# PREDICT-EPFL/piqp

Hardware: AMD Instinct MI355X
Metric: KKT factor+solve/sec (per IPM iter) (higher is better)
Workload: dtype f64; 1 GPU; dense QP n=4096 p=0 m_ineq=4096 (BASELINE configs[1]), kkt_solver=dense_cholesky, 1 update_scalings_and_factor + 2 KKTSystem::solve per step, inputs resident in HBM; n=4096, p=0, m=4096, parallelism=independent QP replicas x1

## Files before the change

piqp_amd/csrc/dense_kernels.hip:

```cpp
#include "dense_kernels.hpp"

#include <algorithm>
#include <map>
#include <mutex>
#include <stdexcept>
#include <type_traits>
#include <utility>
#include <vector>
#include <cstdlib>
#include <cstdio>
#include <cstring>

namespace pq {
namespace dense {

typedef double d4 __attribute__((ext_vector_type(4)));
typedef double d2 __attribute__((ext_vector_type(2)));

__device__ __forceinline__ double readlane_d(double v, int srclane)
{
    long long bits = __double_as_longlong(v);
    int lo = (int)(bits & 0xffffffffll), hi = (int)(bits >> 32);
    lo = __builtin_amdgcn_readlane(lo, srclane);
    hi = __builtin_amdgcn_readlane(hi, srclane);
// ... 595 lines not shown
    if (!front_panel(j, panel, k, nb, rs) || rs <= 0) return;
    const int T = (rs + TS - 1) / TS;
    const int b = (int)blockIdx.x / SPLIT, h = (int)blockIdx.x % SPLIT;
    if (b >= T * (T + 1) / 2) return;
    int ti = (int)((sqrt(8.0 * (double)b + 1.0) - 1.0) * 0.5);
    while ((ti + 1) * (ti + 2) / 2 <= b) ++ti;
    while (ti * (ti + 1) / 2 > b) --ti;
    const int tj = b - ti * (ti + 1) / 2;
    if (ti * TS + (TS / SPLIT) * h >= rs) return;
    SyrkArgs a;
    a.n = rs; a.kdim = nb;
    a.A = j.F + (k + nb) + (size_t)k * j.f; a.lda = j.f; a.B = a.A; a.ldb = j.f; a.w = j.dvec + k;
    a.C = j.F + (k + nb) + (size_t)(k + nb) * j.f; a.ldc = j.f;
    a.unaligned = ((j.f & 1) || (reinterpret_cast<uintptr_t>(a.A) & 15)) ? 1 : 0;
    if (j.multi) {
        a.ncol = j.w - (k + nb);
        if (a.ncol <= 0 || tj * TS >= a.ncol) return;
    }
    extern __shared__ __attribute__((aligned(16))) double smem[];
    (void)fused_tile<512, false, true, true, SPLIT == 4>(a, ti, tj, smem, h);
}

template <int EPI>
__global__ __launch_bounds__(256) void k_syrk_tail_reduce(SyrkArgs a)
{
    const int b = a.tile_begin + (int)blockIdx.x;
    int ti, tj;
    if (a.tile_order) {
        const int pk = a.tile_order[b];
        ti = pk >> 16; tj = pk & 0xffff;
    } else {
        ti = (int)((sqrt(8.0 * (double)b + 1.0) - 1.0) * 0.5);
        while ((ti + 1) * (ti + 2) / 2 <= b) ++ti;
        while (ti * (ti + 1) / 2 > b) --ti;
        tj = b - ti * (ti + 1) / 2;
    }
    const int row0 = ti * TS, col0 = tj * TS;
    const double* P0 = a.part + (size_t)blockIdx.x * a.k_split * TS * TS;
    {
        const int idx = (int)blockIdx.y * 256 + (int)threadIdx.x;
        const int li = idx & (TS - 1), lj = idx >> 7;
        const int gi = row0 + li, gj = col0 + lj;
        if (gi >= a.n || gj >= a.n || gi < gj) return;
        double v = 0.0;
#pragma unroll 8
        for (int sl = 0; sl < a.k_split; ++sl) v += P0[(size_t)sl * TS * TS + idx];
        const size_t ci = (size_t)gi + (size_t)gj * a.ldc;
        if (EPI == EPI_ASSEMBLE) {
            double base = a.Pfull[(size_t)gi + (size_t)gj * a.ldp];
            if (gi == gj) base += a.x_reg[gi];
            if (a.ATA) base += a.dinv * a.ATA[(size_t)gi + (size_t)gj * a.ldata];
            a.C[ci] = base + v;
        } else if (EPI == EPI_SUBTRACT) {
            a.C[ci] -= v;
        } else {
            a.C[ci] = v;
        }
    }
}

static int g_slots = 0;
static int syrk_slots()
{
    if (g_slots == 0) {
        int dev = 0, cus = 256;
        if (hipGetDevice(&dev) == hipSuccess) (void)hipDeviceGetAttribute(&cus, hipDeviceAttributeMultiprocessorCount, dev);
        g_slots = 2 * (cus > 0 ? cus : 256);
    }
    return g_slots;
}
static void syrk_tail_plan(int n, int kdim, int& rem, int& ksplit)
{
    const int T = div_up(n, TS);
    const int ntiles = T * (T + 1) / 2;
    const int slots = syrk_slots();
    const int nkt = div_up(kdim, BK);
    rem = ntiles % slots;
    ksplit = 1;
    if (ntiles > slots && rem > 0 && rem * 10 < slots * 6) {
        int s = slots / rem;
        s = std::min(s, nkt / 4);
        if (s >= 2) ksplit = s;
// ... 12 lines not shown
    bool low_latency;
    bool tile_order;
    int rem, k_split;
};
static bool syrk_wants_tile_order(int T) { return T >= 16; }
static SyrkPlan syrk_plan(int n, int kdim, bool with_ws, size_t ws_doubles)
{
    SyrkPlan p;
    p.T = div_up(n, TS);
    p.ntiles = p.T * (p.T + 1) / 2;
    p.rem = 0; p.k_split = 1;
    if (with_ws) syrk_tail_plan(n, kdim, p.rem, p.k_split);
    if (p.rem > 0 && (size_t)p.rem * p.k_split * TS * TS > ws_doubles) { p.rem = 0; p.k_split = 1; }
    p.low_latency = kdim <= 256;
    p.tile_order = !p.low_latency && syrk_wants_tile_order(p.T);
    return p;
}
void syrk_debug_plan(int n, int kdim, bool with_workspace, int out[6])
{
    const SyrkPlan p = syrk_plan(n, kdim, with_workspace, ~(size_t)0);
    out[0] = p.T; out[1] = p.ntiles; out[2] = p.low_latency ? 1 : 0; out[3] = p.tile_order ? 1 : 0; out[4] = p.rem; out[5] = p.k_split;
}

static const int* syrk_tile_order(int T)
{
    static std::mutex mu;
    static std::map<std::pair<int, int>, int*> cache;
    if (!syrk_wants_tile_order(T)) return nullptr;
    int dev = 0;
    if (hipGetDevice(&dev) != hipSuccess) return nullptr;
    std::lock_guard<std::mutex> lk(mu);
    auto it = cache.find({dev, T});
    if (it != cache.end()) return it->second;
    constexpr int S = 8, NX = 8;
    std::vector<int> blocked;
    for (int SI = 0; SI * S < T; ++SI)
        for (int SJ = 0; SJ <= SI; ++SJ)
            for (int ti = SI * S; ti < std::min(T, SI * S + S); ++ti)
                for (int tj = SJ * S; tj < SJ * S + S && tj <= ti; ++tj) blocked.push_back(ti << 16 | tj);
    const int nt = (int)blocked.size();
    std::vector<int> start(NX + 1, 0);
    for (int x = 0; x < NX; ++x) start[x + 1] = start[x] + nt / NX + (x < nt % NX ? 1 : 0);
    std::vector<int> order(nt);
    for (int b = 0; b < nt; ++b) order[b] = blocked[start[b % NX] + b / NX];
    int* d = nullptr;
    if (hipMalloc(&d, sizeof(int) * nt) != hipSuccess) { (void)hipGetLastError(); cache[{dev, T}] = nullptr; return nullptr; }
    ++alloc_counter();
    if (hipMemcpy(d, order.data(), sizeof(int) * nt, hipMemcpyHostToDevice) != hipSuccess) { (void)hipGetLastError(); (void)hipFree(d); d = nullptr; }
    cache[{dev, T}] = d;
    return d;
}

void syrk_prepare(int n) { (void)syrk_tile_order(div_up(n, TS)); }

template <int EPI>
static void launch_syrk_t(SyrkArgs a, hipStream_t s, double* ws, size_t ws_doubles)
{
    const SyrkPlan pl = syrk_plan(a.n, a.kdim, ws != nullptr, ws_doubles);
    const int main_tiles = pl.ntiles - pl.rem;
    a.tile_begin = 0; a.k_split = 1; a.part = nullptr;
    a.tile_order = pl.tile_order ? syrk_tile_order(pl.T) : nullptr;
    if (pl.low_latency) hipLaunchKernelGGL((k_syrk_lower<EPI, 4, 4>), dim3(main_tiles), dim3(1024), SYRK_LDS_BYTES, s, a);
    else hipLaunchKernelGGL((k_syrk_lower<EPI, 2, 2>), dim3(main_tiles), dim3(256), SYRK_LDS_BYTES, s, a);
    if (pl.rem > 0) {
        a.tile_begin = main_tiles; a.k_split = pl.k_split; a.part = ws;
        hipLaunchKernelGGL((k_syrk_lower<EPI, 2, 2>), dim3(pl.rem * pl.k_split), dim3(256), SYRK_LDS_BYTES, s, a);
        hipLaunchKernelGGL(k_syrk_tail_reduce<EPI>, dim3(pl.rem, TS * TS / 256), dim3(256), 0, s, a);
    }
}

void launch_syrk(int epi, const SyrkArgs& args_in, hipStream_t s, double* split_ws, size_t split_ws_doubles)
{
    SyrkArgs a = args_in;
    if (a.n <= 0) return;
    a.unaligned = ((a.lda & 1) || (a.ldb & 1) || (reinterpret_cast<uintptr_t>(a.A) & 15) || (reinterpret_cast<uintptr_t>(a.B) & 15)) ? 1 : 0;
    static PerDeviceOnce attr_set;
    attr_set([&] {
        PQ_HIP(hipFuncSetAttribute(reinterpret_cast<const void*>(k_syrk_lower<EPI_ASSEMBLE, 2, 2>), hipFuncAttributeMaxDynamicSharedMemorySize, SYRK_LDS_BYTES));
        PQ_HIP(hipFuncSetAttribute(reinterpret_cast<const void*>(k_syrk_lower<EPI_SUBTRACT, 2, 2>), hipFuncAttributeMaxDynamicSharedMemorySize, SYRK_LDS_BYTES));
        PQ_HIP(hipFuncSetAttribute(reinterpret_cast<const void*>(k_syrk_lower<EPI_STORE, 2, 2>), hipFuncAttributeMaxDynamicSharedMemorySize, SYRK_LDS_BYTES));
        PQ_HIP(hipFuncSetAttribute(reinterpret_cast<const void*>(k_syrk_lower<EPI_ASSEMBLE, 4, 4>), hipFuncAttributeMaxDynamicSharedMemorySize, SYRK_LDS_BYTES));
        PQ_HIP(hipFuncSetAttribute(reinterpret_cast<const void*>(k_syrk_lower<EPI_SUBTRACT, 4, 4>), hipFuncAttributeMaxDynamicSharedMemorySize, SYRK_LDS_BYTES));
        PQ_HIP(hipFuncSetAttribute(reinterpret_cast<const void*>(k_syrk_lower<EPI_STORE, 4, 4>), hipFuncAttributeMaxDynamicSharedMemorySize, SYRK_LDS_BYTES));
    });
    if (epi == EPI_SUBTRACT_POTRF) {
        static PerDeviceOnce fused_attr;
        fused_attr([&] {
            PQ_HIP(hipFuncSetAttribute(reinterpret_cast<const void*>(k_syrk_lower<EPI_SUBTRACT_POTRF, 4, 2>), hipFuncAttributeMaxDynamicSharedMemorySize, FUSED_LDS_BYTES));
        });
        const int T = div_up(a.n, TS);
        a.tile_begin = 0; a.k_split = 1; a.part = nullptr;
        if (!a.fuse_scratch || !a.fuse_flags || a.fuse_nb <= 0 || a.kdim > TS) throw std::runtime_error("fused trailing update: scratch / flags / panel width");
        hipLaunchKernelGGL((k_syrk_lower<EPI_SUBTRACT_POTRF, 4, 2>), dim3(T * (T + 1) / 2 + FUSE_ROLES - 1), dim3(512), FUSED_LDS_BYTES, s, a);
        PQ_HIP(hipGetLastError());
        return;
    }
    switch (epi) {
    case EPI_ASSEMBLE: launch_syrk_t<EPI_ASSEMBLE>(a, s, split_ws, split_ws_doubles); break;
    case EPI_SUBTRACT: launch_syrk_t<EPI_SUBTRACT>(a, s, split_ws, split_ws_doubles); break;
    default: launch_syrk_t<EPI_STORE>(a, s, split_ws, split_ws_doubles); break;
    }
    PQ_HIP(hipGetLastError());
}

__global__ __launch_bounds__(256) void k_assemble_no_g(int n, const double* __restrict__ Pf, const double* __restrict__ x_reg, const double* __restrict__ ATA, double dinv, double* __restrict__ C)
{
    const int j = blockIdx.y;
    const int i = blockIdx.x * 256 + threadIdx.x;
    if (i < n && i >= j) {
        double v = Pf[i + (size_t)j * n];
        if (i == j) v += x_reg[i];
        if (ATA) v += dinv * ATA[i + (size_t)j * n];
        C[i + (size_t)j * n] = v;
    }
}
void launch_assemble_no_g(int n, const double* Pf, const double* x_reg, const double* ATA, double dinv, double* C, hipStream_t s)
{
    if (n <= 0) return;
    hipLaunchKernelGGL(k_assemble_no_g, dim3(div_up(n, 256), n), dim3(256), 0, s, n, Pf, x_reg, ATA, dinv, C);
    PQ_HIP(hipGetLastError());
}


// ... 357 lines not shown
    const int tid = threadIdx.x, lane = tid & 63, wave = tid >> 6;
    for (int b = wave; b < TB_BLOCKS; b += POTRF_THREADS / 64) {
        int bi = 0;
        while ((bi + 1) * (bi + 2) / 2 <= b) ++bi;
        const int bj = b - bi * (bi + 1) / 2;
        double v[4];
#pragma unroll
        for (int q = 0; q < 4; ++q) {
            const int e = lane + 64 * q, r = 16 * bi + (e & 15), c = 16 * bj + (e >> 4);
            const bool in = r < nb && c < nb;
            const bool ok = in && r >= c;
            const double* p = ok ? (A + r + (size_t)c * lda) : A;
            const double t = *p;
            v[q] = ok ? t : ((!in && r == c) ? 1.0 : 0.0);
        }
#pragma unroll
        for (int q = 0; q < 4; ++q) Tb[b * 256 + lane + 64 * q] = v[q];
    }
    __syncthreads();
    potrf_block<LDLT, POTRF_THREADS / 64>(Tb, Tb + TB_DOUBLES, nb, kglobal, info, rdiag, dvec, A, lda, pack, w16, ts, cnt, nactive, nullptr, nullptr, 0, nullptr, pack_lkk);
}
template <bool LDLT>
__global__ __launch_bounds__(POTRF_THREADS) void k_potrf_diag(double* __restrict__ A, int lda, int nb, int kglobal, int* __restrict__ info, double* __restrict__ rdiag,
                                                              double* __restrict__ dvec, double* __restrict__ pack, double* __restrict__ w16, long long* __restrict__ ts)
{
    potrf_diag_body<LDLT>(A, lda, nb, kglobal, info, rdiag, dvec, pack, w16, ts);
}
__global__ __launch_bounds__(POTRF_THREADS) void k_potrf_diag_fronts(const FrontJob* __restrict__ jobs, int panel, int* __restrict__ info, double* __restrict__ rdiag)
{
    const FrontJob j = jobs[blockIdx.x];
    int k, nb, rs;
    if (j.kind != 0 || !front_panel(j, panel, k, nb, rs)) return;
    potrf_diag_body<true>(j.F + k + (size_t)k * j.f, j.f, nb, j.first + k, info, rdiag, j.dvec + k, rs > 0 ? j.pack : nullptr, nullptr, nullptr, min(8, (nb + 15) >> 4));
}

void launch_potrf_diag(bool ldlt, double* A, int lda, int nb, int kglobal, int* info, double* rdiag, double* dvec, double* pack, double* w16, hipStream_t s, long long* ts)
{
    static PerDeviceOnce attr_set;
    attr_set([&] {
        PQ_HIP(hipFuncSetAttribute(reinterpret_cast<const void*>(k_potrf_diag<false>), hipFuncAttributeMaxDynamicSharedMemorySize, POTRF_LDS_BYTES));
        PQ_HIP(hipFuncSetAttribute(reinterpret_cast<const void*>(k_potrf_diag<true>), hipFuncAttributeMaxDynamicSharedMemorySize, POTRF_LDS_BYTES));
    });
    if (ldlt) hipLaunchKernelGGL(k_potrf_diag<true>, dim3(1), dim3(POTRF_THREADS), POTRF_LDS_BYTES, s, A, lda, nb, kglobal, info, rdiag, dvec, pack, w16, ts);
    else hipLaunchKernelGGL(k_potrf_diag<false>, dim3(1), dim3(POTRF_THREADS), POTRF_LDS_BYTES, s, A, lda, nb, kglobal, info, rdiag, dvec, pack, w16, ts);
    PQ_HIP(hipGetLastError());
}

template <int NT, bool PERSIST>
__device__ __forceinline__ bool fused_next_diag(const SyrkArgs& a, double* __restrict__ smem, int role)
{
    constexpr int NW = NT / 64;
    static_assert(FUSE_OWN * FUSE_ROLES >= TB_BLOCKS && FUSE_OWN <= NW, "every tile block needs a wave");
    double* As = smem;
    const int tid = threadIdx.x, lane = tid & 63, wave = tid >> 6;
    const int i = lane & 15, g = lane >> 4;
    const bool dbg_ts = FUSE_TS_ON && !PERSIST && a.fuse_ts && tid == 0 && role == 0;
    if (dbg_ts) a.fuse_ts[0] = clock64();
    const int nbn = a.fuse_nb;
    const bool edge = !PERSIST && ((TS > a.n) || a.unaligned);
    const int t = role * FUSE_OWN + wave;
    const bool on = wave < FUSE_OWN && t < TB_BLOCKS;
    int bi = 0;
    {
        const int tt = on ? t : 0;
        while ((bi + 1) * (bi + 2) / 2 <= tt) ++bi;
    }
    const int bj = (on ? t : 0) - bi * (bi + 1) / 2;
// ... 653 lines not shown
    if (hipDeviceGetAttribute(&cus, hipDeviceAttributeMultiprocessorCount, dev) != hipSuccess || cus < 1) { (void)hipGetLastError(); return nullptr; }
    P.grid = std::min<int>(cus * per_cu, (int)h.size());
    if (hipMalloc(&P.tasks, sizeof(CholTask) * h.size()) != hipSuccess) { (void)hipGetLastError(); P.tasks = nullptr; return nullptr; }
    ++alloc_counter();
    if (hipMemcpy(P.tasks, h.data(), sizeof(CholTask) * h.size(), hipMemcpyHostToDevice) != hipSuccess) { (void)hipGetLastError(); (void)hipFree(P.tasks); P.tasks = nullptr; return nullptr; }
    P.ntasks = (int)h.size();
    return &P;
}
int chol_debug_plan(int T, int* out5, int capacity_tasks)
{
    std::vector<CholTask> h;
    chol_build_tasks(T, h);
    if (out5)
        for (size_t q = 0; q < h.size() && (int)q < capacity_tasks; ++q) {
            int* o = out5 + 5 * q;
            o[0] = h[q].kind; o[1] = h[q].round; o[2] = h[q].a; o[3] = h[q].b; o[4] = h[q].gate;
        }
    return (int)h.size();
}
bool chol_persistent_supported(int n) { return n % FACTOR_NB == 0 && n / FACTOR_NB >= 3 && n / FACTOR_NB <= 1024; }
bool chol_prepare(int n) { return chol_persistent_supported(n) && chol_plan(n / FACTOR_NB) != nullptr; }
size_t chol_flag_ints(int n) { const size_t T = (size_t)(n / FACTOR_NB); return 12 + 2 * T * T + 10 * T + 1; }
bool launch_chol_persistent(bool ldlt, double* A, double* side, int lda, int n, int* info, double* rdiag, double* dvec, double* pack2, double* w16, double* scratch, int* fuse_flags, int* fuse_cnt,
                            int token_base, int* flags, int gen, int fcount, hipStream_t s)
{
    const int T = n / FACTOR_NB;
    const CholPlan* P = chol_plan(T);
    if (!P) return false;
    static long long* trace_d = nullptr;
    static size_t trace_n = 0;
    const bool want_trace = debug_token("chol_trace") != nullptr;
    if (want_trace && trace_n < 4 * (size_t)P->ntasks + 64 * (size_t)(T + 1)) {
        if (trace_d) (void)hipFree(trace_d);
        trace_n = 4 * (size_t)P->ntasks + 64 * (size_t)(T + 1);
        PQ_HIP(hipMalloc(&trace_d, trace_n * sizeof(long long)));
    }
    CholArgs c;
    c.A = A; c.side = side; c.lda = lda; c.n = n; c.T = T; c.ldlt = ldlt ? 1 : 0;
    c.info = info; c.rdiag = rdiag; c.dvec = dvec; c.pack2 = pack2; c.w16 = w16;
    c.scratch = scratch; c.fuse_flags = fuse_flags; c.fuse_cnt = fuse_cnt; c.token_base = token_base;
    c.tasks = P->tasks; c.ntasks = P->ntasks;
    c.ticket = flags; c.lready = flags + 12; c.tver = c.lready + (size_t)T * T; c.pdone = c.tver + (size_t)T * T; c.xcnt = c.pdone + T; c.progress = c.xcnt + 8 * (size_t)T; c.dhalf = c.progress + 1;
    c.gen = gen; c.fcount = fcount; c.split_thr = chol_split_thr();
    c.trace = want_trace ? trace_d : nullptr;
    if (want_trace) PQ_HIP(hipMemsetAsync(trace_d, 0, trace_n * sizeof(long long), s));
    PQ_HIP(hipMemsetAsync(flags, 0, 12 * sizeof(int), s));
    hipLaunchKernelGGL(k_chol_persistent, dim3(P->grid), dim3(CHOL_THREADS), FUSED_LDS_BYTES, s, c);
    PQ_HIP(hipGetLastError());
    if (want_trace) {
        std::vector<long long> h(4 * (size_t)P->ntasks + 64 * (size_t)(T + 1));
        std::vector<CholTask> tk((size_t)P->ntasks);
        PQ_HIP(hipMemcpyAsync(h.data(), trace_d, h.size() * sizeof(long long), hipMemcpyDeviceToHost, s));
        PQ_HIP(hipMemcpyAsync(tk.data(), P->tasks, tk.size() * sizeof(CholTask), hipMemcpyDeviceToHost, s));
        stream_wait(s);
        long long t0 = h[0];
        for (int t = 0; t < P->ntasks; ++t) t0 = std::min(t0, h[4 * (size_t)t]);
        auto us = [&](long long v) { return (double)(v - t0) * 0.01; };
        if (const char* fn = std::getenv("PIQP_AMD_CHOL_TRACE_FILE")) {
            if (FILE* fp = std::fopen(fn, "w")) {
                for (int t = 0; t < P->ntasks; ++t)
                    std::fprintf(fp, "%d %d %d %d %d %d %.2f %.2f %.2f %lld\n", t, tk[(size_t)t].kind, tk[(size_t)t].round, tk[(size_t)t].a, tk[(size_t)t].b, tk[(size_t)t].gate, us(h[4 * (size_t)t]),
                                 us(h[4 * (size_t)t + 1]), us(h[4 * (size_t)t + 2]), h[4 * (size_t)t + 3]);
                std::fclose(fp);
            }
        }
        std::fprintf(stderr, "[piqp_amd] k_chol_persistent timeline (us since the first ticket), T = %d, %d tasks, grid %d\n", T, P->ntasks, P->grid);
        for (int k = 0; k + 1 < T; ++k) {
            double own_ready = 0, own_done = 0, help_done = 0, pan_ready = 0, pan_done = 0, bulk_first = 1e30, bulk_last = 0, bulk_work = 0, bulk_wait = 0;
            double r1[3] = {0, 0, 0}, r2[3] = {0, 0, 0}, dg[3] = {0, 0, 0};
// ... 1460 lines not shown
```

piqp_amd/csrc/dense_kernels.hpp:

```cpp
#pragma once

#include "common.hpp"

namespace pq {
namespace dense {

enum { EPI_ASSEMBLE = 0, EPI_SUBTRACT = 1, EPI_STORE = 2, EPI_SUBTRACT_POTRF = 3 };

struct SyrkArgs {
    int n = 0;
    int kdim = 0;
    const double* A = nullptr; int lda = 0;
    const double* B = nullptr; int ldb = 0;
    const double* w = nullptr;
    double* C = nullptr; int ldc = 0;
    const double* Pfull = nullptr; int ldp = 0;
    const double* x_reg = nullptr;
    const double* ATA = nullptr; int ldata = 0;
    double dinv = 0.0;
    int unaligned = 0;
    int ncol = 1 << 30;
    int tile_begin = 0;
    int k_split = 1;
    double* part = nullptr;
// ... 2 lines not shown
    int fuse_nb = 0;
    int fuse_kglobal = 0;
    int fuse_ldlt = 0;
    int* fuse_info = nullptr;
    double* fuse_rdiag = nullptr;
    double* fuse_dvec = nullptr;
    double* fuse_pack = nullptr;
    int fuse_token = 0;
    int* fuse_flags = nullptr;
    double* fuse_scratch = nullptr;
    int* fuse_cnt = nullptr;
    double* fuse_w16 = nullptr;
    int* fuse_xpub = nullptr;
    const int* fuse_xcnt = nullptr;
    double* fuse_side = nullptr;
    long long* fuse_tr2 = nullptr;
    long long* fuse_tr2n = nullptr;
    int* fuse_abort = nullptr;
    const int* late_p[2] = {nullptr, nullptr};
    int late_w[2] = {0, 0};
    long long* fuse_ts = nullptr;
};

void launch_syrk(int epi, const SyrkArgs& args, hipStream_t s, double* split_ws = nullptr, size_t split_ws_doubles = 0);
size_t syrk_split_workspace_doubles(int n, int kdim);
void syrk_debug_plan(int n, int kdim, bool with_workspace, int out[6]);
void syrk_prepare(int n);
void launch_assemble_no_g(int n, const double* Pf, const double* x_reg, const double* ATA, double dinv, double* C, hipStream_t s);
void launch_potrf_diag(bool ldlt, double* A, int lda, int nb, int kglobal, int* info, double* rdiag, double* dvec, double* pack, double* w16, hipStream_t s,
                       long long* ts = nullptr);
double microbench_potrf_block(bool ldlt, int reps, long long* stamps64, hipStream_t s);
int debug_potrf_block(bool ldlt, int nb, int reps, const double* A_host, double* L_host, double* rdiag_host, double* dvec_host, double* pack_host, int* info_host, hipStream_t s);
void launch_trsm_panel(bool ldlt, double* A, int lda, int k0, int nb, int n, const double* pack, const double* rdiag, hipStream_t s);
bool chol_persistent_supported(int n);
bool chol_prepare(int n);
size_t chol_flag_ints(int n);
int chol_debug_plan(int T, int* out5, int capacity_tasks);
bool launch_chol_persistent(bool ldlt, double* A, double* side, int lda, int n, int* info, double* rdiag, double* dvec, double* pack2, double* w16, double* scratch, int* fuse_flags, int* fuse_cnt,
                            int token_base, int* flags, int gen, int fcount, hipStream_t s);
size_t trsv_poll_doubles(int n);
void launch_trsv_poll_init(double* ypoll, int n, hipStream_t s);
void launch_trsv(const double* L, int ld, int n, double* x, const double* rdiag, bool ldlt, double* ypoll, int* ctl, const double* w16, hipStream_t s, long long* ts = nullptr,
                 const double* Vinv = nullptr, int xcd_seq = -1);
bool probe_one_xcd_sweeps(hipStream_t s);
void launch_block_inverse_dd(bool unit, const double* L, int ld, int n, double* Vsq, hipStream_t s);
size_t block_inverse_dd_doubles(int n);
int gemv_n_slices(int rows, int cols);
int launch_gemv_n_partial(int rows, int cols, const double* M, int ld, const double* v, const double* scale, double alpha, double* part, hipStream_t s);
void launch_reduce_partials(int rows, int nslices, const double* part, const double* base, double* y, hipStream_t s);
void launch_gemv_t(int rows, int cols, const double* M, int ld, const double* v, double alpha, double beta, const double* c, const double* sc, double* out, hipStream_t s);
void launch_symmetrize_upper(const double* Pu, int n, double* Pf, double* pdiag, hipStream_t s);
void launch_symmetrize(const double* A, int lda, bool from_lower, int n, double* Pf, double* pdiag, hipStream_t s);
void launch_reciprocal(int n, const double* a, double* out, hipStream_t s);
void launch_flag_nonpositive(int n, const double* rdiag, int* info, hipStream_t s);
double microbench_mfma_f64(int iters, hipStream_t s);
double microbench_hbm_copy(size_t bytes, int iters, hipStream_t s);

constexpr int FACTOR_NB = 128;
constexpr int FACTOR_PACK_DOUBLES = 36 * 256;

struct FrontJob {
    double* F = nullptr;
// ... 16 lines not shown
```

piqp_amd/csrc/dense_kkt.cpp:

```cpp
#include <algorithm>
#include <cstdio>
#include <cstdlib>
#include <stdexcept>
#include <string>
#include <vector>

#include "trace.hpp"
#include "dense_kernels.hpp"
#include "kkt_solver_base.hpp"

namespace pq {

namespace {

class DenseKKT final : public KKTSolverBase {
public:
    DenseKKT(const pq_dense_data* d, int kkt_solver, int device) : dev_(device), n_(d->n), p_(d->p), m_(d->m), ldlt_(kkt_solver == PQ_DENSE_LDLT_NO_PIVOT), st_(device)
    {
        if (n_ <= 0 || p_ < 0 || m_ < 0) throw std::runtime_error("dense KKT: bad dimensions");
        alloc();
        upload(d);
    }

    ~DenseKKT() override
// ... 11 lines not shown
        const_cast<DenseKKT*>(this)->join_inverses();
        stream_wait(st_);
        DenseKKT* k = new DenseKKT(*this, 0);
        return k;
    }

    void update_data_dense(const pq_dense_data* d, int options) override
    {
        (void)options;
        if (d->n != n_ || d->p != p_ || d->m != m_) throw std::runtime_error("update_data: dimension mismatch");
        PQ_HIP(hipSetDevice(dev_));
        upload(d);
    }

    bool update_scalings_and_factor(double delta, const double* x_reg, const double* z_reg) override
    {
        PQ_ZONE("piqp_amd::DenseKKT::update_scalings_and_factor");
        PQ_HIP(hipSetDevice(dev_));
        delta_ = delta;
        join_inverses();
        dense::launch_reciprocal(m_, z_reg, z_reg_inv_.p, st_);
        PQ_HIP(hipMemcpyAsync(x_reg_last_.p, x_reg, sizeof(double) * n_, hipMemcpyDeviceToDevice, st_));
        int t0 = prof_.begin(0, st_);
        update_kkt(x_reg_last_.p, fac_.p);
        prof_.end(0, t0, st_);
        int t1 = prof_.begin(1, st_);
        launch_factor_panels();
        prof_.end(1, t1, st_);
        if (inv_sweeps_) {
            PQ_HIP(hipEventRecord(ev_fac_, st_));
            PQ_HIP(hipStreamWaitEvent(st_inv_, ev_fac_, 0));
            dense::launch_block_inverse_dd(ldlt_, fac_.p, n_, n_, vinv_.p, st_inv_);
            PQ_HIP(hipEventRecord(ev_inv_, st_inv_));
            inv_pending_ = true;
        }
        return factor_status();
    }

    void solve(const double* rhs_x, const double* rhs_y, const double* rhs_z, double* lhs_x, double* lhs_y, double* lhs_z) override
    {
        PQ_ZONE("piqp_amd::DenseKKT::solve");
        PQ_HIP(hipSetDevice(dev_));
        const int tk = prof_.begin(2, st_);
        const double delta_inv = 1.0 / delta_;
        int nsl = 0;
        if (m_ > 0) nsl += dense::launch_gemv_n_partial(n_, m_, GT_.p, n_, rhs_z, z_reg_inv_.p, 1.0, part_.p + (size_t)nsl * n_, st_);
        if (p_ > 0) nsl += dense::launch_gemv_n_partial(n_, p_, AT_.p, n_, rhs_y, nullptr, delta_inv, part_.p + (size_t)nsl * n_, st_);
// ... 44 lines not shown
    {
        PQ_HIP(hipSetDevice(dev_));
        DBuf<double> tmp((size_t)n_ * n_);
        tmp.zero(st_);
        update_kkt(x_reg_last_.p, tmp.p);
        PQ_HIP(hipMemcpyAsync(out_host, tmp.p, sizeof(double) * (size_t)n_ * n_, hipMemcpyDeviceToHost, st_));
        stream_wait(st_);
    }
    void set_profiling(int level) override { prof_.enabled = level != 0; prof_.level = level; }
    void get_profile(int stage, double* total_ms, int* count) override
    {
        if (stage < 0 || stage >= StageProfiler::NSTAGE) throw std::runtime_error("bad stage");
        PQ_HIP(hipSetDevice(dev_));
        prof_.collect(stage, st_, total_ms, count);
    }
    void set_class_failure_semantics(bool on) override { class_semantics_ = on; }
    bool factor_symmetric(const double* A_dev, int lda, bool from_lower) override
    {
        if (p_ != 0 || m_ != 0) throw std::runtime_error("factor_symmetric: a handle with p = m = 0 only");
        PQ_HIP(hipSetDevice(dev_));
        join_inverses();
        delta_ = 1.0;
        dense::launch_symmetrize(A_dev, lda, from_lower, n_, fac_.p, nullptr, st_);
        const int t1 = prof_.begin(1, st_);
        launch_factor_panels();
        prof_.end(1, t1, st_);
        if (inv_sweeps_) {
            PQ_HIP(hipEventRecord(ev_fac_, st_));
            PQ_HIP(hipStreamWaitEvent(st_inv_, ev_fac_, 0));
            dense::launch_block_inverse_dd(ldlt_, fac_.p, n_, n_, vinv_.p, st_inv_);
            PQ_HIP(hipEventRecord(ev_inv_, st_inv_));
            inv_pending_ = true;
        }
        return factor_status();
    }
    void internal_factor(double* out_host) override
    {
        PQ_HIP(hipSetDevice(dev_));
        PQ_HIP(hipMemcpyAsync(out_host, fac_.p, sizeof(double) * (size_t)n_ * n_, hipMemcpyDeviceToHost, st_));
        stream_wait(st_);
    }

private:
    DenseKKT(const DenseKKT& o, int) : dev_(o.dev_), n_(o.n_), p_(o.p_), m_(o.m_), ldlt_(o.ldlt_), class_semantics_(o.class_semantics_), delta_(o.delta_), st_(o.dev_)
    {
        alloc();
// ... 36 lines not shown
            PQ_HIP(hipEventCreateWithFlags(&ev_inv_, hipEventDisableTiming));
        }
        if (debug_token("trsv_ts")) { trsv_ts_.alloc(4 * ((n_ + 127) / 128) + 8); trsv_ts_.zero(st_); }
        if (const char* e = debug_token("fused_ts")) { dbg_panel_ = std::atoi(e); dbg_ts_.alloc(96); dbg_ts_.zero(st_); }
        x_reg_last_.zero(st_);
        fac_.zero(st_);
    }

    void upload(const pq_dense_data* d)
    {
        const size_t nn = (size_t)n_ * n_;
        copy_in(fac_.p, d->P_utri, nn * sizeof(double), d->mem, st_);
        dense::launch_symmetrize_upper(fac_.p, n_, Pfull_.p, Pdiag_.p, st_);
        copy_in(AT_.p, d->AT, (size_t)n_ * p_ * sizeof(double), d->mem, st_);
        copy_in(GT_.p, d->GT, (size_t)n_ * m_ * sizeof(double), d->mem, st_);
        if (p_ > 0) {
            dense::SyrkArgs a;
            a.n = n_; a.kdim = p_; a.A = AT_.p; a.lda = n_; a.B = AT_.p; a.ldb = n_; a.C = ATA_.p; a.ldc = n_;
            dense::launch_syrk(dense::EPI_STORE, a, st_);
        }
        stream_wait(st_);
    }

    void update_kkt(const double* x_reg, double* out)
    {
        const double dinv = 1.0 / delta_;
        if (m_ > 0) {
            dense::launch_syrk(dense::EPI_ASSEMBLE, assembly_args(x_reg, out), st_, split_ws_.p, split_ws_.n);
        } else {
            dense::launch_assemble_no_g(n_, Pfull_.p, x_reg, p_ > 0 ? ATA_.p : nullptr, dinv, out, st_);
        }
    }

    dense::SyrkArgs assembly_args(const double* x_reg, double* out) const
    {
        dense::SyrkArgs a;
        a.n = n_; a.kdim = m_; a.A = GT_.p; a.lda = n_; a.B = GT_.p; a.ldb = n_; a.w = z_reg_inv_.p; a.C = out; a.ldc = n_;
        a.Pfull = Pfull_.p; a.ldp = n_; a.x_reg = x_reg; a.ATA = p_ > 0 ? ATA_.p : nullptr; a.ldata = n_; a.dinv = 1.0 / delta_;
        return a;
    }

    void launch_factor_panels()
    {
        PQ_HIP(hipMemsetAsync(info_.p, 0xFF, sizeof(int), st_));
        const int NB = dense::FACTOR_NB;
        if (chol_persistent_) {
            dense::launch_potrf_diag(ldlt_, fac_.p, n_, NB, 0, info_.p, rdiag_.p, dvec_.p, pack_.p, w16_.p, st_);
            { const int tt = prof_.begin(4, st_); dense::launch_trsm_panel(ldlt_, fac_.p, n_, 0, NB, n_, pack_.p, rdiag_.p, st_); prof_.end(4, tt, st_); }
            const int T = n_ / NB;
            if (chol_gen_ > 0x3fffffff - 2 * (T + 2)) { chol_flags_.zero(st_); chol_gen_ = 0; chol_fcount_ = 0; }
            chol_gen_ += T + 2;
            const int tt = prof_.begin(3, st_);
            if (!dense::launch_chol_persistent(ldlt_, fac_.p, side_.p, n_, n_, info_.p, rdiag_.p, dvec_.p, pack2_.p, w16_.p, fuse_scratch_.p, fuse_flags_.p, fuse_cnt_.p, fuse_token_, chol_flags_.p,
                                               chol_gen_, chol_fcount_, st_))
                throw std::runtime_error("dense factorisation: the persistent launch has no plan for this size / device");
            prof_.end(3, tt, st_);
            fuse_token_ += T - 1;
            ++chol_fcount_;
            return;
        }
        int p = 0;
        for (int k = 0; k < n_; k += NB, ++p) {
            const int nb = (n_ - k < NB) ? n_ - k : NB;
            const int rs = n_ - k - nb;
            double* A11 = fac_.p + k + (size_t)k * n_;
            if (k == 0) dense::launch_potrf_diag(ldlt_, A11, n_, nb, k, info_.p, rdiag_.p, dvec_.p + k, rs > 0 ? pack_.p : nullptr, w16_.p, st_);
            if (rs <= 0) break;
            if (k == 0) { const int tt = prof_.begin(4, st_); dense::launch_trsm_panel(ldlt_, fac_.p, n_, k, nb, n_, pack_.p, rdiag_.p, st_); prof_.end(4, tt, st_); }
            dense::SyrkArgs a;
            a.n = rs; a.kdim = nb;
            a.A = fac_.p + (k + nb) + (size_t)k * n_; a.lda = n_;
            a.B = a.A; a.ldb = n_;
            if (ldlt_) a.w = dvec_.p + k;
            a.C = fac_.p + (k + nb) + (size_t)(k + nb) * n_; a.ldc = n_;
            a.fuse_nb = rs < NB ? rs : NB; a.fuse_kglobal = k + nb; a.fuse_ldlt = ldlt_ ? 1 : 0; a.fuse_info = info_.p; a.fuse_rdiag = rdiag_.p; a.fuse_dvec = dvec_.p + k + nb;
            a.fuse_pack = (rs - a.fuse_nb > 0) ? pack_.p : nullptr;
            a.fuse_w16 = w16_.p + (size_t)((k + nb) / 16) * 256;
            a.fuse_token = ++fuse_token_; a.fuse_flags = fuse_flags_.p; a.fuse_scratch = fuse_scratch_.p; a.fuse_cnt = fuse_cnt_.p;
            a.fuse_ts = (dbg_panel_ == p) ? dbg_ts_.p : nullptr;
            { const int tt = prof_.begin(3, st_); dense::launch_syrk(dense::EPI_SUBTRACT_POTRF, a, st_); prof_.end(3, tt, st_); }
            if (a.fuse_ts) dump_fused_ts(p);
        }
    }
    void dump_fused_ts(int panel)
    {
        long long h[96];
        PQ_HIP(hipMemcpyAsync(h, dbg_ts_.p, sizeof(h), hipMemcpyDeviceToHost, st_));
        stream_wait(st_);
        std::fprintf(stderr, "[piqp_amd] fused panel %d (cycles): C + panel staged %lld, MFMA loop %lld, tiles->LDS %lld, potrf_block %lld; potrf steps (factor/subst/update):", panel, h[4] - h[0], h[1] - h[4], h[2] - h[1], h[3] - h[2]);
        for (int k = 0; k < 8; ++k) std::fprintf(stderr, " %lld/%lld/%lld", h[8 + 8 * k + 1] - h[8 + 8 * k], h[8 + 8 * k + 3] - h[8 + 8 * k + 2], h[8 + 8 * k + 5] - h[8 + 8 * k + 4]);
        std::fprintf(stderr, "\n[piqp_amd]   potrf step start / factored (since launch):");
        for (int k = 0; k < 8; ++k) std::fprintf(stderr, " %lld/%lld", h[8 + 8 * k] - h[0], h[8 + 8 * k + 1] - h[0]);
        std::fprintf(stderr, "; potrf_block end %lld\n[piqp_amd]   first panel workgroup: tile in registers %lld, step k operands seen:", h[3] - h[0], h[80] - h[0]);
        for (int k = 0; k < 8; ++k) std::fprintf(stderr, " %lld", h[72 + k] - h[0]);
        std::fprintf(stderr, ", panel stored %lld\n", h[81] - h[0]);
        std::fprintf(stderr, "[piqp_amd]   an ordinary tile (2, 1): first operand stage in LDS %lld, K loop (incl. the wait for C) %lld, stores drained %lld cycles\n", h[85] - h[84], h[86] - h[85],
                     h[87] - h[86]);
    }
    bool factor_status()
    {
        if (ldlt_ && !class_semantics_) dense::launch_flag_nonpositive(n_, rdiag_.p, info_.p, st_);
        PQ_HIP(hipMemcpyAsync(info_h_.p, info_.p, sizeof(int), hipMemcpyDeviceToHost, st_));
        if (chol_persistent_) PQ_HIP(hipMemcpyAsync(info_h_.p + 1, chol_flags_.p + 1, sizeof(int), hipMemcpyDeviceToHost, st_));
        stream_wait(st_);
        if (chol_persistent_ && info_h_.p[1] != 0) {
            chol_flags_.zero(st_); fuse_cnt_.zero(st_); fuse_flags_.zero(st_);
            chol_gen_ = 0; chol_fcount_ = 0; fuse_token_ = 0;
            stream_wait(st_);
            return false;
        }
        return info_h_.p[0] == -1;
    }

    int dev_, n_, p_, m_;
    bool ldlt_;
    bool class_semantics_ = false;
    double delta_ = 1.0;
    Stream st_, st_inv_;
    DBuf<double> Pfull_, Pdiag_, AT_, GT_, ATA_, fac_, z_reg_inv_, x_reg_last_, dvec_, part_, rdiag_, split_ws_, pack_, w16_, fuse_scratch_;
    DBuf<int> info_, flags_, fuse_flags_, fuse_cnt_, chol_flags_;
    DBuf<double> pack2_, side_;
    bool inv_sweeps_ = false, inv_pending_ = false;
    hipEvent_t ev_fac_ = nullptr, ev_inv_ = nullptr;
    void join_inverses()
    {
        if (!inv_pending_) return;
        PQ_HIP(hipStreamWaitEvent(st_, ev_inv_, 0));
        inv_pending_ = false;
    }
    DBuf<double> vinv_;
    bool chol_persistent_ = false;
    int chol_gen_ = 0, chol_fcount_ = 0;
    int fuse_token_ = 0;
    DBuf<double> ypoll_;
    bool one_xcd_ = false;
    int xcd_seq_ = 0;
    int next_xcd_seq()
    {
        if (!one_xcd_) return -1;
        if (xcd_seq_ >= 50000000) { flags_.zero(st_); xcd_seq_ = 0; }
        return xcd_seq_++;
    }
    HBuf<int> info_h_;
    StageProfiler prof_;
    int dbg_panel_ = -1;
    DBuf<long long> dbg_ts_, trsv_ts_;
    void dump_trsv_ts()
    {
        std::vector<long long> h(trsv_ts_.n);
        PQ_HIP(hipMemcpyAsync(h.data(), trsv_ts_.p, trsv_ts_.bytes(), hipMemcpyDeviceToHost, st_));
        stream_wait(st_);
        std::fprintf(stderr, "[piqp_amd] forward sweep, ticks of the device-wide 100 MHz clock; per block (last producer's values seen -> products / -> solved / -> handed over):");
        const size_t nb = (h.size() - 8) / 4;
        for (size_t r = 1; r < nb; ++r) std::fprintf(stderr, " %lld/%lld/%lld", h[4 * r + 1] - h[4 * r], h[4 * r + 2] - h[4 * r], h[4 * r + 3] - h[4 * r]);
// ... 23 lines not shown
```

Before: 360.8 IPM-iter KKT (1 factor + 2 solves)/s.

## Fold SYRK tail reduce and flag clears into the first potrf_diag launch

The split-K SYRK tail reduction for assembly is deferred and run by extra workgroups of the first diagonal-block Cholesky kernel, provided no tail tile touches the first block column. The info reset memset and the persistent kernel's flag-word memset are also folded into that kernel, with info moved into the chol flags array so factor_status reads abort and info in one copy. This removes several small launches and memsets per factorization. In exchange it adds correctness coupling between the deferred tiles and the diagonal block, and extra grid blocks on the latency-critical potrf kernel.

Measured after the change: 366.0 IPM-iter KKT (1 factor + 2 solves)/s, median of 3. No clear change (+1.4%).

```diff
diff --git a/piqp_amd/csrc/dense_kernels.hip b/piqp_amd/csrc/dense_kernels.hip
--- a/piqp_amd/csrc/dense_kernels.hip
+++ b/piqp_amd/csrc/dense_kernels.hip
@@ -641,9 +641,9 @@
 }
 
 template <int EPI>
-__global__ __launch_bounds__(256) void k_syrk_tail_reduce(SyrkArgs a)
-{
-    const int b = a.tile_begin + (int)blockIdx.x;
+__device__ __forceinline__ void syrk_tail_reduce_element(const SyrkArgs& a, const int tail, const int idx)
+{
+    const int b = a.tile_begin + tail;
     int ti, tj;
     if (a.tile_order) {
         const int pk = a.tile_order[b];
@@ -655,9 +655,8 @@
         tj = b - ti * (ti + 1) / 2;
     }
     const int row0 = ti * TS, col0 = tj * TS;
-    const double* P0 = a.part + (size_t)blockIdx.x * a.k_split * TS * TS;
+    const double* P0 = a.part + (size_t)tail * a.k_split * TS * TS;
     {
-        const int idx = (int)blockIdx.y * 256 + (int)threadIdx.x;
         const int li = idx & (TS - 1), lj = idx >> 7;
         const int gi = row0 + li, gj = col0 + lj;
         if (gi >= a.n || gj >= a.n || gi < gj) return;
@@ -677,6 +676,11 @@
         }
     }
 }
+template <int EPI>
+__global__ __launch_bounds__(256) void k_syrk_tail_reduce(SyrkArgs a)
+{
+    syrk_tail_reduce_element<EPI>(a, (int)blockIdx.x, (int)blockIdx.y * 256 + (int)threadIdx.x);
+}
 
 static int g_slots = 0;
 static int syrk_slots()
@@ -735,16 +739,8 @@
     out[0] = p.T; out[1] = p.ntiles; out[2] = p.low_latency ? 1 : 0; out[3] = p.tile_order ? 1 : 0; out[4] = p.rem; out[5] = p.k_split;
 }
 
-static const int* syrk_tile_order(int T)
-{
-    static std::mutex mu;
-    static std::map<std::pair<int, int>, int*> cache;
-    if (!syrk_wants_tile_order(T)) return nullptr;
-    int dev = 0;
-    if (hipGetDevice(&dev) != hipSuccess) return nullptr;
-    std::lock_guard<std::mutex> lk(mu);
-    auto it = cache.find({dev, T});
-    if (it != cache.end()) return it->second;
+static std::vector<int> syrk_tile_order_host(int T)
+{
     constexpr int S = 8, NX = 8;
     std::vector<int> blocked;
     for (int SI = 0; SI * S < T; ++SI)
@@ -756,6 +752,45 @@
     for (int x = 0; x < NX; ++x) start[x + 1] = start[x] + nt / NX + (x < nt % NX ? 1 : 0);
     std::vector<int> order(nt);
     for (int b = 0; b < nt; ++b) order[b] = blocked[start[b % NX] + b / NX];
+    return order;
+}
+static bool syrk_tail_avoids_first_column(const SyrkPlan& pl)
+{
+    static std::mutex mu;
+    static std::map<std::pair<int, int>, bool> cache;
+    std::lock_guard<std::mutex> lk(mu);
+    const auto key = std::make_pair(pl.T, pl.rem);
+    auto it = cache.find(key);
+    if (it != cache.end()) return it->second;
+    bool& ok = cache[key];
+    ok = false;
+    const std::vector<int> order = pl.tile_order ? syrk_tile_order_host(pl.T) : std::vector<int>();
+    for (int b = pl.ntiles - pl.rem; b < pl.ntiles; ++b) {
+        int tj;
+        if (pl.tile_order) tj = order[(size_t)b] & 0xffff;
+        else {
+            int ti = (int)((std::sqrt(8.0 * (double)b + 1.0) - 1.0) * 0.5);
+            while ((ti + 1) * (ti + 2) / 2 <= b) ++ti;
+            while (ti * (ti + 1) / 2 > b) --ti;
+            tj = b - ti * (ti + 1) / 2;
+        }
+        if (tj == 0) return false;
+    }
+    ok = true;
+    return true;
+}
+static const int* syrk_tile_order(int T)
+{
+    static std::mutex mu;
+    static std::map<std::pair<int, int>, int*> cache;
+    if (!syrk_wants_tile_order(T)) return nullptr;
+    int dev = 0;
+    if (hipGetDevice(&dev) != hipSuccess) return nullptr;
+    std::lock_guard<std::mutex> lk(mu);
+    auto it = cache.find({dev, T});
+    if (it != cache.end()) return it->second;
+    const std::vector<int> order = syrk_tile_order_host(T);
+    const int nt = (int)order.size();
     int* d = nullptr;
     if (hipMalloc(&d, sizeof(int) * nt) != hipSuccess) { (void)hipGetLastError(); cache[{dev, T}] = nullptr; return nullptr; }
     ++alloc_counter();
@@ -767,10 +802,12 @@
 void syrk_prepare(int n) { (void)syrk_tile_order(div_up(n, TS)); }
 
 template <int EPI>
-static void launch_syrk_t(SyrkArgs a, hipStream_t s, double* ws, size_t ws_doubles)
-{
+static void launch_syrk_t(SyrkArgs a, hipStream_t s, double* ws, size_t ws_doubles, SyrkTailReduce* defer)
+{
+    static const bool reduce_launch = debug_token("syrk_reduce_launch") != nullptr;
     const SyrkPlan pl = syrk_plan(a.n, a.kdim, ws != nullptr, ws_doubles);
     const int main_tiles = pl.ntiles - pl.rem;
+    if (defer) defer->rem = 0;
     a.tile_begin = 0; a.k_split = 1; a.part = nullptr;
     a.tile_order = pl.tile_order ? syrk_tile_order(pl.T) : nullptr;
     if (pl.low_latency) hipLaunchKernelGGL((k_syrk_lower<EPI, 4, 4>), dim3(main_tiles), dim3(1024), SYRK_LDS_BYTES, s, a);
@@ -778,12 +815,14 @@
     if (pl.rem > 0) {
         a.tile_begin = main_tiles; a.k_split = pl.k_split; a.part = ws;
         hipLaunchKernelGGL((k_syrk_lower<EPI, 2, 2>), dim3(pl.rem * pl.k_split), dim3(256), SYRK_LDS_BYTES, s, a);
-        hipLaunchKernelGGL(k_syrk_tail_reduce<EPI>, dim3(pl.rem, TS * TS / 256), dim3(256), 0, s, a);
-    }
-}
-
-void launch_syrk(int epi, const SyrkArgs& args_in, hipStream_t s, double* split_ws, size_t split_ws_doubles)
-{
+        if (EPI == EPI_ASSEMBLE && defer && !reduce_launch && syrk_tail_avoids_first_column(pl)) { defer->a = a; defer->rem = pl.rem; }
+        else hipLaunchKernelGGL(k_syrk_tail_reduce<EPI>, dim3(pl.rem, TS * TS / 256), dim3(256), 0, s, a);
+    }
+}
+
+void launch_syrk(int epi, const SyrkArgs& args_in, hipStream_t s, double* split_ws, size_t split_ws_doubles, SyrkTailReduce* defer)
+{
+    if (defer) defer->rem = 0;
     SyrkArgs a = args_in;
     if (a.n <= 0) return;
     a.unaligned = ((a.lda & 1) || (a.ldb & 1) || (reinterpret_cast<uintptr_t>(a.A) & 15) || (reinterpret_cast<uintptr_t>(a.B) & 15)) ? 1 : 0;
@@ -809,9 +848,9 @@
         return;
     }
     switch (epi) {
-    case EPI_ASSEMBLE: launch_syrk_t<EPI_ASSEMBLE>(a, s, split_ws, split_ws_doubles); break;
-    case EPI_SUBTRACT: launch_syrk_t<EPI_SUBTRACT>(a, s, split_ws, split_ws_doubles); break;
-    default: launch_syrk_t<EPI_STORE>(a, s, split_ws, split_ws_doubles); break;
+    case EPI_ASSEMBLE: launch_syrk_t<EPI_ASSEMBLE>(a, s, split_ws, split_ws_doubles, defer); break;
+    case EPI_SUBTRACT: launch_syrk_t<EPI_SUBTRACT>(a, s, split_ws, split_ws_doubles, nullptr); break;
+    default: launch_syrk_t<EPI_STORE>(a, s, split_ws, split_ws_doubles, nullptr); break;
     }
     PQ_HIP(hipGetLastError());
 }
@@ -1215,8 +1254,17 @@
 }
 template <bool LDLT>
 __global__ __launch_bounds__(POTRF_THREADS) void k_potrf_diag(double* __restrict__ A, int lda, int nb, int kglobal, int* __restrict__ info, double* __restrict__ rdiag,
-                                                              double* __restrict__ dvec, double* __restrict__ pack, double* __restrict__ w16, long long* __restrict__ ts)
-{
+                                                              double* __restrict__ dvec, double* __restrict__ pack, double* __restrict__ w16, long long* __restrict__ ts,
+                                                              int reset_info, int* __restrict__ clear_words, SyrkArgs red, int red_rem)
+{
+    if (blockIdx.x > 0) {
+        constexpr int PER_TILE = TS * TS / POTRF_THREADS;
+        const int q = (int)blockIdx.x - 1;
+        if (q / PER_TILE < red_rem) syrk_tail_reduce_element<EPI_ASSEMBLE>(red, q / PER_TILE, (q % PER_TILE) * POTRF_THREADS + (int)threadIdx.x);
+        return;
+    }
+    if (clear_words && threadIdx.x < 12 && clear_words + threadIdx.x != info) clear_words[threadIdx.x] = 0;
+    if (reset_info && threadIdx.x == 0) *info = -1;
     potrf_diag_body<LDLT>(A, lda, nb, kglobal, info, rdiag, dvec, pack, w16, ts);
 }
 __global__ __launch_bounds__(POTRF_THREADS) void k_potrf_diag_fronts(const FrontJob* __restrict__ jobs, int panel, int* __restrict__ info, double* __restrict__ rdiag)
@@ -1227,15 +1275,19 @@
     potrf_diag_body<true>(j.F + k + (size_t)k * j.f, j.f, nb, j.first + k, info, rdiag, j.dvec + k, rs > 0 ? j.pack : nullptr, nullptr, nullptr, min(8, (nb + 15) >> 4));
 }
 
-void launch_potrf_diag(bool ldlt, double* A, int lda, int nb, int kglobal, int* info, double* rdiag, double* dvec, double* pack, double* w16, hipStream_t s, long long* ts)
-{
+void launch_potrf_diag(bool ldlt, double* A, int lda, int nb, int kglobal, int* info, double* rdiag, double* dvec, double* pack, double* w16, hipStream_t s, long long* ts,
+                       bool reset_info, int* clear_words, const SyrkTailReduce* reduce)
+{
+    const int red_rem = reduce ? reduce->rem : 0;
+    const SyrkArgs red = red_rem > 0 ? reduce->a : SyrkArgs();
+    const dim3 grid(1 + red_rem * (TS * TS / POTRF_THREADS));
     static PerDeviceOnce attr_set;
     attr_set([&] {
         PQ_HIP(hipFuncSetAttribute(reinterpret_cast<const void*>(k_potrf_diag<false>), hipFuncAttributeMaxDynamicSharedMemorySize, POTRF_LDS_BYTES));
         PQ_HIP(hipFuncSetAttribute(reinterpret_cast<const void*>(k_potrf_diag<true>), hipFuncAttributeMaxDynamicSharedMemorySize, POTRF_LDS_BYTES));
     });
-    if (ldlt) hipLaunchKernelGGL(k_potrf_diag<true>, dim3(1), dim3(POTRF_THREADS), POTRF_LDS_BYTES, s, A, lda, nb, kglobal, info, rdiag, dvec, pack, w16, ts);
-    else hipLaunchKernelGGL(k_potrf_diag<false>, dim3(1), dim3(POTRF_THREADS), POTRF_LDS_BYTES, s, A, lda, nb, kglobal, info, rdiag, dvec, pack, w16, ts);
+    if (ldlt) hipLaunchKernelGGL(k_potrf_diag<true>, grid, dim3(POTRF_THREADS), POTRF_LDS_BYTES, s, A, lda, nb, kglobal, info, rdiag, dvec, pack, w16, ts, reset_info ? 1 : 0, clear_words, red, red_rem);
+    else hipLaunchKernelGGL(k_potrf_diag<false>, grid, dim3(POTRF_THREADS), POTRF_LDS_BYTES, s, A, lda, nb, kglobal, info, rdiag, dvec, pack, w16, ts, reset_info ? 1 : 0, clear_words, red, red_rem);
     PQ_HIP(hipGetLastError());
 }
 
@@ -1935,7 +1987,7 @@
 bool chol_prepare(int n) { return chol_persistent_supported(n) && chol_plan(n / FACTOR_NB) != nullptr; }
 size_t chol_flag_ints(int n) { const size_t T = (size_t)(n / FACTOR_NB); return 12 + 2 * T * T + 10 * T + 1; }
 bool launch_chol_persistent(bool ldlt, double* A, double* side, int lda, int n, int* info, double* rdiag, double* dvec, double* pack2, double* w16, double* scratch, int* fuse_flags, int* fuse_cnt,
-                            int token_base, int* flags, int gen, int fcount, hipStream_t s)
+                            int token_base, int* flags, int gen, int fcount, hipStream_t s, bool words_cleared)
 {
     const int T = n / FACTOR_NB;
     const CholPlan* P = chol_plan(T);
@@ -1957,7 +2009,7 @@
     c.gen = gen; c.fcount = fcount; c.split_thr = chol_split_thr();
     c.trace = want_trace ? trace_d : nullptr;
     if (want_trace) PQ_HIP(hipMemsetAsync(trace_d, 0, trace_n * sizeof(long long), s));
-    PQ_HIP(hipMemsetAsync(flags, 0, 12 * sizeof(int), s));
+    if (!words_cleared) PQ_HIP(hipMemsetAsync(flags, 0, 12 * sizeof(int), s));
     hipLaunchKernelGGL(k_chol_persistent, dim3(P->grid), dim3(CHOL_THREADS), FUSED_LDS_BYTES, s, c);
     PQ_HIP(hipGetLastError());
     if (want_trace) {
diff --git a/piqp_amd/csrc/dense_kernels.hpp b/piqp_amd/csrc/dense_kernels.hpp
--- a/piqp_amd/csrc/dense_kernels.hpp
+++ b/piqp_amd/csrc/dense_kernels.hpp
@@ -48,22 +48,28 @@
     long long* fuse_ts = nullptr;
 };
 
-void launch_syrk(int epi, const SyrkArgs& args, hipStream_t s, double* split_ws = nullptr, size_t split_ws_doubles = 0);
+struct SyrkTailReduce {
+    SyrkArgs a;
+    int rem = 0;
+};
+void launch_syrk(int epi, const SyrkArgs& args, hipStream_t s, double* split_ws = nullptr, size_t split_ws_doubles = 0, SyrkTailReduce* defer = nullptr);
 size_t syrk_split_workspace_doubles(int n, int kdim);
 void syrk_debug_plan(int n, int kdim, bool with_workspace, int out[6]);
 void syrk_prepare(int n);
 void launch_assemble_no_g(int n, const double* Pf, const double* x_reg, const double* ATA, double dinv, double* C, hipStream_t s);
 void launch_potrf_diag(bool ldlt, double* A, int lda, int nb, int kglobal, int* info, double* rdiag, double* dvec, double* pack, double* w16, hipStream_t s,
-                       long long* ts = nullptr);
+                       long long* ts = nullptr,
+                       bool reset_info = false, int* clear_words = nullptr, const SyrkTailReduce* reduce = nullptr);
 double microbench_potrf_block(bool ldlt, int reps, long long* stamps64, hipStream_t s);
 int debug_potrf_block(bool ldlt, int nb, int reps, const double* A_host, double* L_host, double* rdiag_host, double* dvec_host, double* pack_host, int* info_host, hipStream_t s);
 void launch_trsm_panel(bool ldlt, double* A, int lda, int k0, int nb, int n, const double* pack, const double* rdiag, hipStream_t s);
 bool chol_persistent_supported(int n);
 bool chol_prepare(int n);
 size_t chol_flag_ints(int n);
+constexpr int CHOL_ABORT_WORD = 1, CHOL_INFO_WORD = 2;
 int chol_debug_plan(int T, int* out5, int capacity_tasks);
 bool launch_chol_persistent(bool ldlt, double* A, double* side, int lda, int n, int* info, double* rdiag, double* dvec, double* pack2, double* w16, double* scratch, int* fuse_flags, int* fuse_cnt,
-                            int token_base, int* flags, int gen, int fcount, hipStream_t s);
+                            int token_base, int* flags, int gen, int fcount, hipStream_t s, bool words_cleared = false);
 size_t trsv_poll_doubles(int n);
 void launch_trsv_poll_init(double* ypoll, int n, hipStream_t s);
 void launch_trsv(const double* L, int ld, int n, double* x, const double* rdiag, bool ldlt, double* ypoll, int* ctl, const double* w16, hipStream_t s, long long* ts = nullptr,
diff --git a/piqp_amd/csrc/dense_kkt.cpp b/piqp_amd/csrc/dense_kkt.cpp
--- a/piqp_amd/csrc/dense_kkt.cpp
+++ b/piqp_amd/csrc/dense_kkt.cpp
@@ -57,7 +57,7 @@
         dense::launch_reciprocal(m_, z_reg, z_reg_inv_.p, st_);
         PQ_HIP(hipMemcpyAsync(x_reg_last_.p, x_reg, sizeof(double) * n_, hipMemcpyDeviceToDevice, st_));
         int t0 = prof_.begin(0, st_);
-        update_kkt(x_reg_last_.p, fac_.p);
+        update_kkt(x_reg_last_.p, fac_.p, &tail_reduce_);
         prof_.end(0, t0, st_);
         int t1 = prof_.begin(1, st_);
         launch_factor_panels();
@@ -148,6 +148,7 @@
         join_inverses();
         delta_ = 1.0;
         dense::launch_symmetrize(A_dev, lda, from_lower, n_, fac_.p, nullptr, st_);
+        tail_reduce_.rem = 0;
         const int t1 = prof_.begin(1, st_);
         launch_factor_panels();
         prof_.end(1, t1, st_);
@@ -230,11 +231,12 @@
         stream_wait(st_);
     }
 
-    void update_kkt(const double* x_reg, double* out)
+    void update_kkt(const double* x_reg, double* out, dense::SyrkTailReduce* defer = nullptr)
     {
         const double dinv = 1.0 / delta_;
+        if (defer) defer->rem = 0;
         if (m_ > 0) {
-            dense::launch_syrk(dense::EPI_ASSEMBLE, assembly_args(x_reg, out), st_, split_ws_.p, split_ws_.n);
+            dense::launch_syrk(dense::EPI_ASSEMBLE, assembly_args(x_reg, out), st_, split_ws_.p, split_ws_.n, defer);
         } else {
             dense::launch_assemble_no_g(n_, Pfull_.p, x_reg, p_ > 0 ? ATA_.p : nullptr, dinv, out, st_);
         }
@@ -250,17 +252,18 @@
 
     void launch_factor_panels()
     {
-        PQ_HIP(hipMemsetAsync(info_.p, 0xFF, sizeof(int), st_));
         const int NB = dense::FACTOR_NB;
+        const dense::SyrkTailReduce reduce = tail_reduce_;
+        tail_reduce_.rem = 0;
         if (chol_persistent_) {
-            dense::launch_potrf_diag(ldlt_, fac_.p, n_, NB, 0, info_.p, rdiag_.p, dvec_.p, pack_.p, w16_.p, st_);
-            { const int tt = prof_.begin(4, st_); dense::launch_trsm_panel(ldlt_, fac_.p, n_, 0, NB, n_, pack_.p, rdiag_.p, st_); prof_.end(4, tt, st_); }
             const int T = n_ / NB;
             if (chol_gen_ > 0x3fffffff - 2 * (T + 2)) { chol_flags_.zero(st_); chol_gen_ = 0; chol_fcount_ = 0; }
+            dense::launch_potrf_diag(ldlt_, fac_.p, n_, NB, 0, info_dev(), rdiag_.p, dvec_.p, pack_.p, w16_.p, st_, nullptr, true, chol_flags_.p, &reduce);
+            { const int tt = prof_.begin(4, st_); dense::launch_trsm_panel(ldlt_, fac_.p, n_, 0, NB, n_, pack_.p, rdiag_.p, st_); prof_.end(4, tt, st_); }
             chol_gen_ += T + 2;
             const int tt = prof_.begin(3, st_);
-            if (!dense::launch_chol_persistent(ldlt_, fac_.p, side_.p, n_, n_, info_.p, rdiag_.p, dvec_.p, pack2_.p, w16_.p, fuse_scratch_.p, fuse_flags_.p, fuse_cnt_.p, fuse_token_, chol_flags_.p,
-                                               chol_gen_, chol_fcount_, st_))
+            if (!dense::launch_chol_persistent(ldlt_, fac_.p, side_.p, n_, n_, info_dev(), rdiag_.p, dvec_.p, pack2_.p, w16_.p, fuse_scratch_.p, fuse_flags_.p, fuse_cnt_.p, fuse_token_, chol_flags_.p,
+                                               chol_gen_, chol_fcount_, st_, true))
                 throw std::runtime_error("dense factorisation: the persistent launch has no plan for this size / device");
             prof_.end(3, tt, st_);
             fuse_token_ += T - 1;
@@ -272,7 +275,7 @@
             const int nb = (n_ - k < NB) ? n_ - k : NB;
             const int rs = n_ - k - nb;
             double* A11 = fac_.p + k + (size_t)k * n_;
-            if (k == 0) dense::launch_potrf_diag(ldlt_, A11, n_, nb, k, info_.p, rdiag_.p, dvec_.p + k, rs > 0 ? pack_.p : nullptr, w16_.p, st_);
+            if (k == 0) dense::launch_potrf_diag(ldlt_, A11, n_, nb, k, info_dev(), rdiag_.p, dvec_.p + k, rs > 0 ? pack_.p : nullptr, w16_.p, st_, nullptr, true, nullptr, &reduce);
             if (rs <= 0) break;
             if (k == 0) { const int tt = prof_.begin(4, st_); dense::launch_trsm_panel(ldlt_, fac_.p, n_, k, nb, n_, pack_.p, rdiag_.p, st_); prof_.end(4, tt, st_); }
             dense::SyrkArgs a;
@@ -281,7 +284,7 @@
             a.B = a.A; a.ldb = n_;
             if (ldlt_) a.w = dvec_.p + k;
             a.C = fac_.p + (k + nb) + (size_t)(k + nb) * n_; a.ldc = n_;
-            a.fuse_nb = rs < NB ? rs : NB; a.fuse_kglobal = k + nb; a.fuse_ldlt = ldlt_ ? 1 : 0; a.fuse_info = info_.p; a.fuse_rdiag = rdiag_.p; a.fuse_dvec = dvec_.p + k + nb;
+            a.fuse_nb = rs < NB ? rs : NB; a.fuse_kglobal = k + nb; a.fuse_ldlt = ldlt_ ? 1 : 0; a.fuse_info = info_dev(); a.fuse_rdiag = rdiag_.p; a.fuse_dvec = dvec_.p + k + nb;
             a.fuse_pack = (rs - a.fuse_nb > 0) ? pack_.p : nullptr;
             a.fuse_w16 = w16_.p + (size_t)((k + nb) / 16) * 256;
             a.fuse_token = ++fuse_token_; a.fuse_flags = fuse_flags_.p; a.fuse_scratch = fuse_scratch_.p; a.fuse_cnt = fuse_cnt_.p;
@@ -305,19 +308,28 @@
         std::fprintf(stderr, "[piqp_amd]   an ordinary tile (2, 1): first operand stage in LDS %lld, K loop (incl. the wait for C) %lld, stores drained %lld cycles\n", h[85] - h[84], h[86] - h[85],
                      h[87] - h[86]);
     }
+    int* info_dev() { return chol_persistent_ ? chol_flags_.p + dense::CHOL_INFO_WORD : info_.p; }
     bool factor_status()
     {
-        if (ldlt_ && !class_semantics_) dense::launch_flag_nonpositive(n_, rdiag_.p, info_.p, st_);
-        PQ_HIP(hipMemcpyAsync(info_h_.p, info_.p, sizeof(int), hipMemcpyDeviceToHost, st_));
-        if (chol_persistent_) PQ_HIP(hipMemcpyAsync(info_h_.p + 1, chol_flags_.p + 1, sizeof(int), hipMemcpyDeviceToHost, st_));
-        stream_wait(st_);
-        if (chol_persistent_ && info_h_.p[1] != 0) {
+        static_assert(dense::CHOL_INFO_WORD == dense::CHOL_ABORT_WORD + 1, "factor_status reads the two words with one copy");
+        if (ldlt_ && !class_semantics_) dense::launch_flag_nonpositive(n_, rdiag_.p, info_dev(), st_);
+        int abort_word = 0, info = -1;
+        if (chol_persistent_) {
+            PQ_HIP(hipMemcpyAsync(info_h_.p, chol_flags_.p + dense::CHOL_ABORT_WORD, 2 * sizeof(int), hipMemcpyDeviceToHost, st_));
+            stream_wait(st_);
+            abort_word = info_h_.p[0]; info = info_h_.p[1];
+        } else {
+            PQ_HIP(hipMemcpyAsync(info_h_.p, info_.p, sizeof(int), hipMemcpyDeviceToHost, st_));
+            stream_wait(st_);
+            info = info_h_.p[0];
+        }
+        if (abort_word != 0) {
             chol_flags_.zero(st_); fuse_cnt_.zero(st_); fuse_flags_.zero(st_);
             chol_gen_ = 0; chol_fcount_ = 0; fuse_token_ = 0;
             stream_wait(st_);
             return false;
         }
-        return info_h_.p[0] == -1;
+        return info == -1;
     }
 
     int dev_, n_, p_, m_;
@@ -338,6 +350,7 @@
     }
     DBuf<double> vinv_;
     bool chol_persistent_ = false;
+    dense::SyrkTailReduce tail_reduce_;
     int chol_gen_ = 0, chol_fcount_ = 0;
     int fuse_token_ = 0;
     DBuf<double> ypoll_;
```
